# etiiiR/pixel-nerf

Measured on AMD Instinct MI355X. Metric: rays/sec (coarse+fine, 64+64 samples), higher is better.
Workload: dtype f32 (f16x3)

## Files before the change

### pixel-nerf_amd/csrc/mlp_dev.h

```cpp
#pragma once
#include "pnr_diag.h"
#include <cstddef>
#include <type_traits>

#include "mlp_layout.h"

namespace pnr {
namespace mlpk {

__device__ __forceinline__ f4 mfma(float a, float b, f4 c) {
    return __builtin_amdgcn_mfma_f32_16x16x4f32(a, b, c, 0, 0, 0);
}

typedef f4 Acc[RTW][CT];

__device__ __forceinline__ int opaque_lane(int lane) {
    asm volatile("" : "+v"(lane));
    return lane;
}

__device__ __forceinline__ void save_relu(const Acc &acc, float *slot, int64_t tile, int64_t n_points,
                                          int wave, int lane) {
    lane = opaque_lane(lane);
    const int g = lane >> 4, cl = lane & 15;
#pragma unroll
    for (int c = 0; c < CT; ++c) {
        const int64_t p = tile * COLS + 16 * c + cl;
        if (p >= n_points) continue;
#pragma unroll
        for (int r = 0; r < RTW; ++r) {
            const f4 v = acc[r][c];
            *reinterpret_cast<f4 *>(slot + p * H + 16 * (RTW * wave + r) + 4 * g) = relu4(v);
        }
    }
}

__device__ __forceinline__ void save_mask(const Acc &acc, uint32_t *mslot, int64_t tile, int64_t n_points,
                                          int wave, int lane) {
    static_assert(RTW == 4, "mask bytes assume 4 row tiles per wave");
    lane = opaque_lane(lane);
    const int g = lane >> 4, cl = lane & 15;
    auto nib = [](const f4 &v) {
        return (v.x > 0.f ? 1u : 0u) | (v.y > 0.f ? 2u : 0u) | (v.z > 0.f ? 4u : 0u) | (v.w > 0.f ? 8u : 0u);
    };
#pragma unroll
    for (int c = 0; c < CT; ++c) {
        const int64_t p = tile * COLS + 16 * c + cl;
        const uint32_t bits = nib(acc[0][c]) | (nib(acc[1][c]) << 4) | (nib(acc[2][c]) << 8) | (nib(acc[3][c]) << 12);
        if (p < n_points)
            *reinterpret_cast<uint16_t *>(reinterpret_cast<char *>(mslot) + p * 64 + 8 * wave + 2 * g) =
                (uint16_t)bits;
    }
}

template <int NK>
__device__ __forceinline__ void gemm(Acc &acc, const float *__restrict__ wp, const float *inb) {
    f4 A[RTW], B[CT];
#pragma unroll
    for (int r = 0; r < RTW; ++r) A[r] = *reinterpret_cast<const f4 *>(wp + r * 256);
#pragma unroll
    for (int c = 0; c < CT; ++c) B[c] = *reinterpret_cast<const f4 *>(inb + c * 16 * LDS_LD);
#pragma unroll 2
    for (int kb = 0; kb < NK; ++kb) {
        f4 An[RTW], Bn[CT];
        const int kn = kb + 1 < NK ? kb + 1 : kb;
#pragma unroll
        for (int r = 0; r < RTW; ++r)
            An[r] = *reinterpret_cast<const f4 *>(wp + (int64_t)kn * KB_FLOATS + r * 256);
#pragma unroll
        for (int c = 0; c < CT; ++c)
            Bn[c] = *reinterpret_cast<const f4 *>(inb + c * 16 * LDS_LD + kn * 16);
#pragma unroll
        for (int j = 0; j < 4; ++j)
#pragma unroll
            for (int c = 0; c < CT; ++c)
#pragma unroll
                for (int r = 0; r < RTW; ++r) acc[r][c] = mfma(A[r][j], B[c][j], acc[r][c]);
#pragma unroll
        for (int r = 0; r < RTW; ++r) A[r] = An[r];
#pragma unroll
        for (int c = 0; c < CT; ++c) B[c] = Bn[c];
    }
}

typedef float f8 __attribute__((ext_vector_type(8)));

__device__ __forceinline__ void split3(const f4 &lo, const f4 &hi, bf8 &x0, bf8 &x1, bf8 &x2) {
    const float x[8] = {lo.x, lo.y, lo.z, lo.w, hi.x, hi.y, hi.z, hi.w};
    u4 p0, p1, p2;
#pragma unroll
    for (int q = 0; q < 4; ++q) {
        unsigned a, b, c;
        split_pair(x[2 * q], x[2 * q + 1], a, b, c);
        p0[q] = a;
        p1[q] = b;
        p2[q] = c;
    }
    x0 = __builtin_bit_cast(bf8, p0);
    x1 = __builtin_bit_cast(bf8, p1);
    x2 = __builtin_bit_cast(bf8, p2);
}

__device__ __forceinline__ void lds_barrier() {
    asm volatile("s_waitcnt lgkmcnt(0)\n\ts_barrier" ::: "memory");
}

constexpr int A_DIST = 3;
constexpr int A_RING = A_DIST < 4 ? 4 : 8;

template <int NKS, int NTERM>
__device__ __forceinline__ void gemm_split(Acc &acc, const float *__restrict__ wp, const float *inbw,
                                           float *stg, int wave, int lane) {
    bf8 ra[A_RING][3];
    auto loadA = [&](bf8 (&dst)[3], int ks, int r) {
        const float *src = wp + (int64_t)ks * SKS_FLOATS + r * SRT_FLOATS;
#pragma unroll
        for (int q = 0; q < 3; ++q) dst[q] = *reinterpret_cast<const bf8 *>(src + q * 256);
    };
    auto split_own = [&](int ks, int buf) {
        const float *bp = inbw + 32 * ks;
        const f4 v = *reinterpret_cast<const f4 *>(bp);
        unsigned a0, a1, a2, b0, b1, b2;
        split_pair(v.x, v.y, a0, a1, a2);
        split_pair(v.z, v.w, b0, b1, b2);
        typedef unsigned u2 __attribute__((ext_vector_type(2)));
        float *d = stg + buf * STG_FLOATS + (wave % CT) * 768 + lane * 4 + 2 * (wave / CT);
        *reinterpret_cast<u2 *>(d) = u2{a0, b0};
        *reinterpret_cast<u2 *>(d + 256) = u2{a1, b1};
        *reinterpret_cast<u2 *>(d + 512) = u2{a2, b2};
    };
    split_own(0, 0);
#pragma unroll
    for (int r = 0; r < A_DIST; ++r) loadA(ra[r], 0, r);
    lds_barrier();
#pragma unroll 1
    for (int ks = 0; ks < NKS; ++ks) {
        const int kn = ks + 1 < NKS ? ks + 1 : ks;
        bf8 b0[CT], b1[CT], b2[CT];
        const float *sp = stg + (ks & 1) * STG_FLOATS + lane * 4;
#pragma unroll
        for (int c = 0; c < CT; ++c) {
            b0[c] = *reinterpret_cast<const bf8 *>(sp + c * 768);
            b1[c] = *reinterpret_cast<const bf8 *>(sp + c * 768 + 256);
            b2[c] = *reinterpret_cast<const bf8 *>(sp + c * 768 + 512);
        }
#pragma unroll
        for (int r = 0; r < RTW; ++r) {
            if (r == 1) split_own(kn, (ks + 1) & 1);
            const int rn = r + A_DIST;
            if (rn < RTW) loadA(ra[rn % A_RING], ks, rn);
            else loadA(ra[rn % A_RING], kn, rn - RTW);
            __builtin_amdgcn_sched_barrier(0);
            const bf8 *a = ra[r % A_RING];
#pragma unroll
            for (int c = 0; c < CT; ++c) {
                f4 v = acc[r][c];
                if (NTERM >= 9) {
                    v = mfma_bf(a[2], b2[c], v);
                    v = mfma_bf(a[1], b2[c], v);
                    v = mfma_bf(a[2], b1[c], v);
                }
                v = mfma_bf(a[2], b0[c], v);
                v = mfma_bf(a[1], b1[c], v);
                v = mfma_bf(a[0], b2[c], v);
                v = mfma_bf(a[1], b0[c], v);
                v = mfma_bf(a[0], b1[c], v);
                v = mfma_bf(a[0], b0[c], v);
                acc[r][c] = v;
            }
        }
        lds_barrier();
    }
}

typedef _Float16 h2 __attribute__((ext_vector_type(2)));
typedef float f2 __attribute__((ext_vector_type(2)));
typedef unsigned u2 __attribute__((ext_vector_type(2)));

__device__ __forceinline__ void split_f16x4(const f4 &v, float s, u2 &p0, u2 &p1) {
    const f2 a = {v.x * s, v.y * s}, b = {v.z * s, v.w * s};
    const unsigned a0 = __builtin_bit_cast(unsigned, __builtin_convertvector(a, h2));
    const unsigned b0 = __builtin_bit_cast(unsigned, __builtin_convertvector(b, h2));
    p0 = u2{a0, b0};
    p1 = u2{resid_pk(a0, a.x, a.y), resid_pk(b0, b.x, b.y)};
}

__device__ __forceinline__ int swz(int col, int k) {
    return 8 * ((k >> 3) ^ ((col >> 2) & 3)) + (k & 7);
}

template <int DIST, int NP = 2>
struct HRing {
    static constexpr int slots = DIST < RTW ? RTW : 2 * RTW;
    h8 ra[slots][NP];
};

template <int DIST, int NP>
__device__ __forceinline__ void hring_load(HRing<DIST, NP> &R, const float *__restrict__ wp, int slot, int ks, int r) {
    const float *src = wp + (int64_t)ks * sks_h_floats(NP) + r * srt_h_floats(NP);
    R.ra[slot][0] = *reinterpret_cast<const h8 *>(src);
    if constexpr (NP > 1) R.ra[slot][1] = *reinterpret_cast<const h8 *>(src + 256);
}

template <int DIST, int NKS = KS32, int NP = 2>
__device__ __forceinline__ void hring_prime(HRing<DIST, NP> &R, const float *__restrict__ wp) {
#pragma unroll
    for (int t = 0; t < DIST; ++t) hring_load(R, wp, t, (t / RTW) & (NKS - 1), t % RTW);
}

struct Fair {
    int *prog;
    int wave, it, mate;
};
template <int NKS, int DIST = H_DIST, int NP = 2>
__device__ __forceinline__ void gemm_f16_primed(Acc &acc, HRing<DIST, NP> &R, const float *__restrict__ wp,
                                                const _Float16 *pb0, const _Float16 *pb1, Fair *F = nullptr) {
    constexpr int H_RING = HRing<DIST, NP>::slots;
    static_assert(DIST < H_RING && H_RING % RTW == 0, "ring");
    constexpr int U = H_RING / RTW;
    static_assert(NKS % U == 0, "k-steps");
    static_assert((NKS & (NKS - 1)) == 0, "rotation mask");
    auto kstep = [&](int ks, auto ph_tag, auto tail_tag) {
        constexpr int ph = decltype(ph_tag)::value;
        constexpr bool tail = decltype(tail_tag)::value;
        h8 b0[CT], b1[CT];
        const int kr = ks & (NKS - 1);
#pragma unroll
        for (int c = 0; c < CT; ++c) {
            b0[c] = *reinterpret_cast<const h8 *>(pb0 + c * 16 * ROWH + 32 * kr);
            if constexpr (NP > 1) b1[c] = *reinterpret_cast<const h8 *>(pb1 + c * 16 * ROWH + 32 * kr);
        }
#pragma unroll
        for (int r = 0; r < RTW; ++r) {
            const int tn = ph * RTW + r + DIST;
            if (!tail || tn < U * RTW)
                hring_load(R, wp, tn % H_RING, (ks - ph + tn / RTW) & (NKS - 1), tn % RTW);
            __builtin_amdgcn_sched_barrier(0);
            const h8 *a = R.ra[(ph * RTW + r) % H_RING];
#pragma unroll
            for (int c = 0; c < CT; ++c) {
                f4 v = acc[r][c];
                if constexpr (NP > 1) {
                    v = mfma_h(a[1], b0[c], v);
                    v = mfma_h(a[0], b1[c], v);
                }
                v = mfma_h(a[0], b0[c], v);
                acc[r][c] = v;
            }
        }
    };
    auto iter = [&](int ks0, auto tail_tag) {
        if (F) {
            const int it = ++F->it;
            if (it > __builtin_amdgcn_readfirstlane(F->mate)) __builtin_amdgcn_s_setprio(0);
            else __builtin_amdgcn_s_setprio(1);
            F->prog[F->wave] = it;
            F->mate = F->prog[F->wave ^ 4];
        }
        kstep(ks0, std::integral_constant<int, 0>{}, tail_tag);
        if constexpr (U > 1) kstep(ks0 + 1, std::integral_constant<int, 1>{}, tail_tag);
    };
#pragma unroll 1
    for (int ks = 0; ks + U < NKS; ks += U) iter(ks, std::false_type{});
    iter(NKS - U, std::true_type{});
    if (F) __builtin_amdgcn_s_setprio(0);
}

template <int NKS, int DIST = H_DIST, int NP = 2>
__device__ __forceinline__ void gemm_f16(Acc &acc, const float *__restrict__ wp, const _Float16 *pb0,
                                         const _Float16 *pb1, Fair *F = nullptr) {
    HRing<DIST, NP> R;
    hring_prime<DIST, NKS, NP>(R, wp);
    gemm_f16_primed<NKS, DIST, NP>(acc, R, wp, pb0, pb1, F);
}

__device__ __forceinline__ void put_split4(_Float16 *P0, _Float16 *P1, int off, const f4 &v, float s) {
    u2 p0, p1;
    split_f16x4(v, s, p0, p1);
    *reinterpret_cast<u2 *>(P0 + off) = p0;
    *reinterpret_cast<u2 *>(P1 + off) = p1;
}

template <bool RELU = true>
__device__ __forceinline__ void relu_colmax(const Acc &acc, float *cmax, int wave, int lane) {
    lane = opaque_lane(lane);
    const int g = lane >> 4, cl = lane & 15;
#pragma unroll
    for (int c = 0; c < CT; ++c) {
        float m = 0.f;
#pragma unroll
        for (int r = 0; r < RTW; ++r) {
            f4 v = acc[r][c];
            if constexpr (!RELU) v = f4{fabsf(v.x), fabsf(v.y), fabsf(v.z), fabsf(v.w)};
            m = max3_nc(max3_nc(m, v.x, v.y), v.z, v.w);
        }
        m = rows_max(m);
        if (g == 0) cmax[(16 * c + cl) * 8 + wave] = m;
    }
}

__device__ __forceinline__ void put_split4_pair(_Float16 *Pl, int off, const f4 &v, float s) {
    u2 p0, p1;
    split_f16x4(v, s, p0, p1);
    const auto w0 = __builtin_amdgcn_permlane16_swap(p0.x, p1.x, false, false);
    const auto w1 = __builtin_amdgcn_permlane16_swap(p0.y, p1.y, false, false);
    typedef unsigned u4 __attribute__((ext_vector_type(4)));
    *reinterpret_cast<u4 *>(Pl + off) = u4{w0[0], w1[0], w0[1], w1[1]};
}
__device__ __forceinline__ void put_f16x4_pair(_Float16 *q, int off, const f4 &va, const f4 &vb, float s) {
    const f2 a0 = {va.x * s, va.y * s}, a1 = {va.z * s, va.w * s};
    const f2 b0 = {vb.x * s, vb.y * s}, b1 = {vb.z * s, vb.w * s};
    const u2 pa = {__builtin_bit_cast(unsigned, __builtin_convertvector(a0, h2)),
                   __builtin_bit_cast(unsigned, __builtin_convertvector(a1, h2))};
    const u2 pb = {__builtin_bit_cast(unsigned, __builtin_convertvector(b0, h2)),
                   __builtin_bit_cast(unsigned, __builtin_convertvector(b1, h2))};
    const auto w0 = __builtin_amdgcn_permlane16_swap(pa.x, pb.x, false, false);
    const auto w1 = __builtin_amdgcn_permlane16_swap(pa.y, pb.y, false, false);
    typedef unsigned u4 __attribute__((ext_vector_type(4)));
    *reinterpret_cast<u4 *>(q + off) = u4{w0[0], w1[0], w0[1], w1[1]};
}
template <bool RELU = true, int NP = 2>
__device__ __forceinline__ void relu_store_split(const Acc &acc, _Float16 *P0, _Float16 *P1,
                                                 const float *cmax, int *ecol, int wave, int lane,
                                                 int (&e_col)[CT]) {
    lane = opaque_lane(lane);
    const int g = lane >> 4, cl = lane & 15;
    _Float16 *Pl = (NP > 1 && (g & 1)) ? P1 : P0;
    const int kb = 16 * RTW * wave + 4 * (g & ~1);
    _Float16 *q0 = Pl + cl * ROWH + swz(cl, kb), *q1 = Pl + cl * ROWH + swz(cl, kb + 16);
#pragma unroll
    for (int c = 0; c < CT; ++c) {
        const int col = 16 * c + cl;
        const f4 m0 = *reinterpret_cast<const f4 *>(cmax + col * 8);
        const f4 m1 = *reinterpret_cast<const f4 *>(cmax + col * 8 + 4);
        e_col[c] = scale_exp(max3_nc(max3_nc(m0.x, m0.y, m0.z), max3_nc(m0.w, m1.x, m1.y), max_nc(m1.z, m1.w)));
    }
    if (wave == 0 && g == 0) {
#pragma unroll
        for (int c = 0; c < CT; ++c) ecol[16 * c + cl] = e_col[c];
    }
#pragma unroll
    for (int c = 0; c < CT; ++c) {
        const int col = 16 * c + cl;
        const float sc = __builtin_ldexpf(1.f, e_col[c]);
        if constexpr (NP == 1) {
            static_assert(RTW % 2 == 0, "row-tile pairs");
#pragma unroll
            for (int j = 0; j < RTW / 2; ++j) {
                const f4 va = RELU ? relu4(acc[2 * j][c]) : acc[2 * j][c];
                const f4 vb = RELU ? relu4(acc[2 * j + 1][c]) : acc[2 * j + 1][c];
                put_f16x4_pair((g & 1) ? q1 : q0, c * 16 * ROWH + j * 32, va, vb, sc);
            }
        } else {
#pragma unroll
        for (int r = 0; r < RTW; ++r) {
            const f4 v = acc[r][c];
            const f4 o = RELU ? relu4(v) : v;
            put_split4_pair((r & 1) ? q1 : q0, c * 16 * ROWH + (r >> 1) * 32, o, sc);
        }
        }
    }
}

__device__ __forceinline__ void load_bias(f4 (&b)[RTW], const float *__restrict__ bias, int wave, int lane) {
    const int g = opaque_lane(lane) >> 4;
#pragma unroll
    for (int r = 0; r < RTW; ++r) b[r] = *reinterpret_cast<const f4 *>(bias + 16 * (RTW * wave + r) + 4 * g);
}
__device__ __forceinline__ void set_bias(Acc &acc, const f4 (&b)[RTW], bool accumulate) {
#pragma unroll
    for (int r = 0; r < RTW; ++r)
#pragma unroll
        for (int c = 0; c < CT; ++c) acc[r][c] = accumulate ? acc[r][c] + b[r] : b[r];
}

__device__ __forceinline__ void add_bias(Acc &acc, const float *__restrict__ bias, int wave, int lane,
                                         bool accumulate) {
    const int g = opaque_lane(lane) >> 4;
#pragma unroll
    for (int r = 0; r < RTW; ++r) {
        const f4 b = *reinterpret_cast<const f4 *>(bias + 16 * (RTW * wave + r) + 4 * g);
#pragma unroll
        for (int c = 0; c < CT; ++c) acc[r][c] = accumulate ? acc[r][c] + b : b;
    }
}

__device__ __forceinline__ void store_relu(const Acc &acc, float *inbuf, int wave, int lane) {
    const int g = lane >> 4, cl = lane & 15;
#pragma unroll
    for (int r = 0; r < RTW; ++r)
#pragma unroll
        for (int c = 0; c < CT; ++c) {
            const f4 v = acc[r][c];
            const f4 o = relu4(v);
            *reinterpret_cast<f4 *>(inbuf + (16 * c + cl) * LDS_LD + 16 * (RTW * wave + r) + 4 * g) = o;
        }
}

#ifdef PNR_PHASE_TIMING
constexpr int PT_SLOTS = 20;
#endif

struct GemmCtx {
    int64_t wl_off, ws_off;
    const float *inb4;
    const float *inbw;
    float *stg;
    const float *hdr;
    const _Float16 *pb0, *pb1;
    const int *ecol;
    int ecl[CT];
    Fair fair;
    int wave, lane;
#ifdef PNR_PHASE_TIMING
    uint64_t pt[PT_SLOTS], pt_last;
#endif
};

struct CellRows {
    f4 c[2][4];
};
__device__ __forceinline__ void cell_load(CellRows &C, const float *__restrict__ pz, const float *gtab, int cj,
                                          int lane) {
    const f4 to = *reinterpret_cast<const f4 *>(gtab + cj * 8);
#pragma unroll
    for (int half = 0; half < 2; ++half) {
        const uint32_t ch = half * 256 + opaque_lane(lane) * 4;
        C.c[half][0] = *reinterpret_cast<const f4 *>(pz + __float_as_uint(to.x) + ch);
        C.c[half][1] = *reinterpret_cast<const f4 *>(pz + __float_as_uint(to.y) + ch);
        C.c[half][2] = *reinterpret_cast<const f4 *>(pz + __float_as_uint(to.z) + ch);
        C.c[half][3] = *reinterpret_cast<const f4 *>(pz + __float_as_uint(to.w) + ch);
    }
}
__device__ __forceinline__ void cell_blend_store(const CellRows &C, const float *gtab, float *stage, int cj,
                                                 int lane) {
    const f4 tw = *reinterpret_cast<const f4 *>(gtab + cj * 8 + 4);
#pragma unroll
    for (int half = 0; half < 2; ++half) {
        const uint32_t ch = half * 256 + opaque_lane(lane) * 4;
        const f4 *c = C.c[half];
        f4 zz;
#pragma unroll
        for (int q = 0; q < 4; ++q)
            zz[q] = add_rn(add_rn(add_rn(mul_rn(c[0][q], tw.x), mul_rn(c[1][q], tw.y)), mul_rn(c[2][q], tw.z)),
                           mul_rn(c[3][q], tw.w));
        *reinterpret_cast<f4 *>(stage + cj * LDS_LD + ch) = zz;
    }
}
__device__ __forceinline__ uint32_t cell_run_starts(const float *gtab, int c0) {
    uint32_t starts = 1u;
    uint32_t prev = __builtin_amdgcn_readfirstlane(__float_as_uint(gtab[c0 * 8]));
#pragma unroll
    for (int j = 1; j < COLS / WAVES; ++j) {
        const uint32_t k = __builtin_amdgcn_readfirstlane(__float_as_uint(gtab[(c0 + j) * 8]));
        if (k != prev) starts |= 1u << j;
        prev = k;
    }
    return starts;
}
__device__ __forceinline__ void stage_proj_runs(const float *__restrict__ pz, const float *gtab, float *stage,
                                                int wave, int lane) {
    constexpr int NC = COLS / WAVES;
    const int c0 = NC * wave;
    const uint32_t starts = cell_run_starts(gtab, c0);
    auto next = [&](int j) -> int {
        const uint32_t m = starts & ~((2u << j) - 1u);
        return m ? __builtin_ctz(m) : NC;
    };
    CellRows A, B, C;
    int a = 0, b = next(0), c = b < NC ? next(b) : NC;
    cell_load(A, pz, gtab, c0 + a, lane);
    if (b < NC) cell_load(B, pz, gtab, c0 + b, lane);
    if (c < NC) cell_load(C, pz, gtab, c0 + c, lane);
    lds_barrier();
    int j = 0;
    for (;;) {
        const int d = c < NC ? next(c) : NC;
        for (; j < b; ++j) cell_blend_store(A, gtab, stage, c0 + j, lane);
        if (j >= NC) break;
        if (d < NC) cell_load(A, pz, gtab, c0 + d, lane);
        const int e = d < NC ? next(d) : NC;
        for (; j < c; ++j) cell_blend_store(B, gtab, stage, c0 + j, lane);
        if (j >= NC) break;
        if (e < NC) cell_load(B, pz, gtab, c0 + e, lane);
        const int f = e < NC ? next(e) : NC;
        for (; j < d; ++j) cell_blend_store(C, gtab, stage, c0 + j, lane);
        if (j >= NC) break;
        if (f < NC) cell_load(C, pz, gtab, c0 + f, lane);
        a = d;
        b = e;
        c = f;
    }
}
template <bool HP>
__device__ __forceinline__ void stage_latent_gather(const float *__restrict__ latent, const float *gtab, float *image,
                                                    _Float16 *P0, _Float16 *P1, int *ecol, float *zsave,
                                                    int64_t n_valid, int wave, int lane) {
#pragma unroll 4
    for (int j = 0; j < COLS / WAVES; ++j) {
        const int cj = (COLS / WAVES) * wave + j;
        const f4 to = *reinterpret_cast<const f4 *>(gtab + cj * 8);
        const f4 tw = *reinterpret_cast<const f4 *>(gtab + cj * 8 + 4);
        f4 zh[2];
#pragma unroll
        for (int half = 0; half < 2; ++half) {
            const uint32_t ch = half * 256 + opaque_lane(lane) * 4;
            const f4 c0 = *reinterpret_cast<const f4 *>(latent + __float_as_uint(to.x) + ch);
            const f4 c1 = *reinterpret_cast<const f4 *>(latent + __float_as_uint(to.y) + ch);
            const f4 c2 = *reinterpret_cast<const f4 *>(latent + __float_as_uint(to.z) + ch);
            const f4 c3 = *reinterpret_cast<const f4 *>(latent + __float_as_uint(to.w) + ch);
            f4 zz;
#pragma unroll
            for (int q = 0; q < 4; ++q)
                zz[q] = add_rn(add_rn(add_rn(mul_rn(c0[q], tw.x), mul_rn(c1[q], tw.y)), mul_rn(c2[q], tw.z)),
                               mul_rn(c3[q], tw.w));
            if constexpr (HP) zh[half] = zz;
            else *reinterpret_cast<f4 *>(image + cj * LDS_LD + ch) = zz;
            if (zsave && cj < n_valid) *reinterpret_cast<f4 *>(zsave + (int64_t)cj * H + ch) = zz;
        }
        if constexpr (HP) {
            float m = 0.f;
#pragma unroll
            for (int hf = 0; hf < 2; ++hf)
                m = fmaxf(m, fmaxf(fmaxf(fabsf(zh[hf][0]), fabsf(zh[hf][1])), fmaxf(fabsf(zh[hf][2]), fabsf(zh[hf][3]))));
            m = wave_max(m);
            const int e = scale_exp(m);
            const float sc = __builtin_ldexpf(1.f, e);
            put_split4(P0, P1, cj * ROWH + swz(cj, lane * 4), zh[0], sc);
            put_split4(P0, P1, cj * ROWH + swz(cj, 256 + lane * 4), zh[1], sc);
            if (lane == 0) ecol[cj] = e;
        }
    }
}
__device__ __forceinline__ void add_stage(Acc &x, const float *stage, int wave, int lane) {
    lane = opaque_lane(lane);
    const int g = lane >> 4, cl = lane & 15;
#pragma unroll
    for (int r = 0; r < RTW; ++r)
#pragma unroll
        for (int c = 0; c < CT; ++c) {
            const f4 v = *reinterpret_cast<const f4 *>(stage + (16 * c + cl) * LDS_LD + 16 * (RTW * wave + r) + 4 * g);
            f4 o;
#pragma unroll
            for (int q = 0; q < 4; ++q) o[q] = add_rn(x[r][c][q], v[q]);
            x[r][c] = o;
        }
}

template <int PREC, int NK, int DIST = H_DIST, bool OWN = false, int NP = nparts(PREC)>
__device__ __forceinline__ void layer_gemm(Acc &acc, const float *layer_base, GemmCtx &g, int hidx,
                                           HRing<DIST, NP> *R = nullptr) {
    PT(g, 3);
    PT_COUNT(g, 5);
    if constexpr (PREC == 0) {
        gemm<NK>(acc, layer_base + g.wl_off, g.inb4);
    } else if constexpr (is_h(PREC)) {
        const int cl = opaque_lane(g.lane) & 15;
        const int ew = (int)g.hdr[HDR_ESCALE + hidx];
        float sa[CT], ia[CT];
#pragma unroll
        for (int c = 0; c < CT; ++c) {
            const int e = (OWN ? g.ecl[c] : g.ecol[16 * c + cl]) + ew;
            sa[c] = __builtin_ldexpf(1.f, e);
            ia[c] = __builtin_ldexpf(1.f, -e);
        }
#pragma unroll
        for (int r = 0; r < RTW; ++r)
#pragma unroll
            for (int c = 0; c < CT; ++c) {
                acc[r][c] *= sa[c];
            }
        Fair *F = g.fair.prog ? &g.fair : nullptr;
        const int wso = NP == nparts(PREC) ? (int)g.ws_off : RTW * g.wave * srt_h_floats(NP) + g.lane * 4;
        if (R) gemm_f16_primed<NK / 2, DIST, NP>(acc, *R, layer_base + opaque_lane(wso), g.pb0, g.pb1, F);
        else gemm_f16<NK / 2, DIST, NP>(acc, layer_base + opaque_lane(wso), g.pb0, g.pb1, F);
#pragma unroll
        for (int r = 0; r < RTW; ++r)
#pragma unroll
            for (int c = 0; c < CT; ++c) {
                acc[r][c] *= ia[c];
            }
    } else {
        gemm_split<NK / 2, PREC>(acc, layer_base + g.ws_off, g.inbw, g.stg, g.wave, g.lane);
    }
    PT(g, 2);
}

__device__ __forceinline__ int claim_one(int *p) {
    int old;
    unsigned long long saved;
    asm volatile(
        "s_mov_b64 %1, exec\n\t"
        "s_mov_b64 exec, 1\n\t"
        "s_nop 4\n\t"
        "global_atomic_add %0, %2, %3, off sc0\n\t"
        "s_mov_b64 exec, %1\n\t"
        "s_waitcnt vmcnt(0)\n\t"
        "s_nop 4"
        : "=&v"(old), "=&s"(saved)
        : "v"(p), "v"(1)
        : "memory");
    return __builtin_amdgcn_readfirstlane(old);
}

}
}
```

### pixel-nerf_amd/csrc/mlp_layout.h

```cpp
#pragma once
#include "pnr_common.h"

namespace pnr {
namespace mlpk {

constexpr int H = 512;
constexpr int NRT = H / 16;
constexpr int NKB = H / 16;
constexpr int NKB_IN = 4;
constexpr int WAVES = 8;
constexpr int NTHR = 64 * WAVES;
constexpr int RTW = NRT / WAVES;
constexpr int CT = 4;
constexpr int COLS = 16 * CT;
constexpr int LDS_LD = H + 4;
constexpr int KB_FLOATS = NRT * 256;
constexpr int LAYER_FLOATS = NKB * KB_FLOATS;
constexpr int HDR = 64;
constexpr int KS32 = H / 32;
constexpr int KS32_IN = 2;
constexpr int SRT_FLOATS = 768;
constexpr int SKS_FLOATS = NRT * SRT_FLOATS;
constexpr int SRT16_FLOATS = 512;
constexpr int SKS16_FLOATS = NRT * SRT16_FLOATS;
constexpr int HDR_ESCALE = 32;
__host__ __device__ constexpr bool is_h(int prec) { return prec == 3 || prec == 1; }
__host__ __device__ constexpr int nparts(int prec) { return prec == 1 ? 1 : 2; }
__host__ __device__ constexpr int srt_h_floats(int np) { return np * 256; }
__host__ __device__ constexpr int sks_h_floats(int np) { return NRT * srt_h_floats(np); }
static_assert(srt_h_floats(2) == SRT16_FLOATS && sks_h_floats(2) == SKS16_FLOATS, "two-part layout");
__host__ __device__ constexpr int sks_floats(int prec) {
    return prec == 3 ? SKS16_FLOATS : prec == 1 ? sks_h_floats(1) : SKS_FLOATS;
}
__host__ __device__ constexpr int sks_in_floats(int prec) { return is_h(prec) ? SKS16_FLOATS : SKS_FLOATS; }
constexpr int STG_FLOATS = CT * 3 * 256;
constexpr int ROWH = H + 16;
constexpr int PART_HALVES = COLS * ROWH;
constexpr int H_DIST = 4;

struct Layout {
    int prec;
    int n_linz, n_l512, n_blocks, ncomb, d_in, d_out, pe_n;
    int64_t layer_floats;
    int64_t off_lin_in, off_l512, off_lin_out, off_bias, nbias, off_out32, total;
};

inline Layout make_layout(const pnr_mlp_desc &d) {
    Layout L;
    L.n_blocks = d.n_blocks;
    L.n_linz = d.combine_layer < d.n_blocks ? d.combine_layer : d.n_blocks;
    L.ncomb = L.n_linz;
    L.n_l512 = L.n_linz + 2 * d.n_blocks;
    L.d_in = d.d_in;
    L.d_out = d.d_out;
    L.pe_n = d.pe_n;
    L.prec = d.precision;
    L.layer_floats = L.prec ? (int64_t)KS32 * sks_floats(L.prec) : (int64_t)LAYER_FLOATS;
    L.off_lin_in = HDR;
    L.off_l512 = L.off_lin_in + (L.prec ? (int64_t)KS32_IN * sks_in_floats(L.prec) : (int64_t)NKB_IN * KB_FLOATS);
    L.off_lin_out = L.off_l512 + (int64_t)L.n_l512 * L.layer_floats;
    L.off_bias = L.off_lin_out + (int64_t)NKB * 256;
    L.nbias = (int64_t)(1 + L.n_l512) * H + 16;
    L.off_out32 = ((L.off_bias + L.nbias + 63) / 64) * 64;
    L.total = L.off_out32 + (is_h(L.prec) ? 4 * H : 0);
    return L;
}

__host__ __device__ inline int layer_index(int blk, int kind, int n_linz) {
    return blk < n_linz ? 3 * blk + kind : 3 * n_linz + 2 * (blk - n_linz) + (kind - 1);
}

__host__ __device__ constexpr int64_t save_floats_per_point(int n_blocks) {
    return 64 + (int64_t)H * (2 + 2 * n_blocks) + 16 * (2 * n_blocks + 1);
}
__host__ __device__ constexpr int64_t save_mask_offset(int n_blocks, int64_t n_points) {
    return (64 + (int64_t)H * (2 + 2 * n_blocks)) * n_points;
}

__device__ __forceinline__ int scale_exp(float m) {
    if (!(m > 0.f) || !(m < 3.0e38f)) return 0;
    int e = 14 - __builtin_amdgcn_frexp_expf(m);
    return e < -64 ? -64 : (e > 40 ? 40 : e);
}

struct FwdLds {
    int stg, gtab, cmax, ecol, petab, s_next, prog, hpart, mreg, mscr, mnf, petab_f, end, ltab;
};
enum LeanTab { LT_END = 0, LT_LSTEP, LT_STEP, LT_PAD, LT_WLF, LT_HLF, LT_KX, LT_KY, LT_HX, LT_HY, LT_FLOATS = 16 };
constexpr int IMG_H_FLOATS = PART_HALVES;
constexpr int MARCH_BUF_FLOATS = 640;
constexpr FwdLds fwd_lds(bool hp) {
    FwdLds m = {};
    m.stg = COLS * LDS_LD;
    m.gtab = hp ? IMG_H_FLOATS : m.stg + 2 * STG_FLOATS;
    m.cmax = m.gtab + COLS * 8;
    m.ecol = m.cmax + COLS * 8;
    m.petab = hp ? m.ecol + COLS : m.gtab + COLS * 8;
    m.s_next = m.petab + 32;
    m.prog = m.petab + 40;
    m.hpart = m.petab + 64;
    m.mreg = hp ? m.hpart + WAVES * COLS * 4 : m.petab + 36;
    m.mscr = m.mreg + MARCH_BUF_FLOATS;
    m.mnf = m.mscr + 3 * 128;
    m.petab_f = m.mnf + 4;
    m.end = m.petab_f + 32;
    m.ltab = m.end;
    return m;
}
constexpr size_t lds_bytes(const FwdLds &m, bool march) { return sizeof(float) * (size_t)(march ? m.end : m.mreg); }
constexpr size_t lds_bytes_lean(const FwdLds &m) { return sizeof(float) * (size_t)(m.ltab + LT_FLOATS); }
constexpr int MARCH_LDS_FLOATS = fwd_lds(true).end - fwd_lds(true).mreg;

struct BwdLds {
    int cmax, ecol, prog, end;
};
constexpr BwdLds bwd_lds() {
    BwdLds m = {};
    m.cmax = IMG_H_FLOATS;
    m.ecol = m.cmax + COLS * 8;
    m.prog = m.ecol + COLS;
    m.end = m.prog + WAVES;
    return m;
}
constexpr size_t lds_bytes(const BwdLds &m) { return sizeof(float) * (size_t)m.end; }

static_assert(lds_bytes(fwd_lds(true), false) == 147968 && lds_bytes(fwd_lds(false), false) == 158864 &&
              lds_bytes(bwd_lds()) == 137504, "LDS totals");
static_assert(lds_bytes(fwd_lds(true), true) == 147968 + 4 * MARCH_LDS_FLOATS &&
              lds_bytes(fwd_lds(false), true) == 158864 + 4 * MARCH_LDS_FLOATS &&
              fwd_lds(false).end - fwd_lds(false).mreg == MARCH_LDS_FLOATS, "LDS totals with the march region");
static_assert(lds_bytes(fwd_lds(true), true) <= 160 * 1024 && lds_bytes(fwd_lds(false), true) <= 160 * 1024 &&
              lds_bytes(bwd_lds()) <= 160 * 1024, "one workgroup's LDS");
static_assert(lds_bytes_lean(fwd_lds(true)) == lds_bytes(fwd_lds(true), true) + 4 * LT_FLOATS &&
              lds_bytes_lean(fwd_lds(true)) <= 160 * 1024 && fwd_lds(true).ltab % 4 == 0,
              "the lean table fits beside the fp16 map and the march region, 16-byte aligned");
static_assert(sizeof(float) * COLS * LDS_LD <= 2 * sizeof(_Float16) * PART_HALVES,
              "the fp32 stage fits in the split image it aliases");

}
}
```

### pixel-nerf_amd/csrc/mlp_pack.hip

```cpp
#include "mlp_layout.h"
#include "pnr_launch.h"

namespace pnr {
namespace mlpk {

struct PackSrc {
    const float *lin_in_w, *lin_in_b, *lin_out_w, *lin_out_b, *pe_f, *pe_p;
    const float *w[24], *b[24];
};

__global__ void k_pack(PackSrc s, Layout L, float *__restrict__ out) {
    const int64_t i = (int64_t)blockIdx.x * blockDim.x + threadIdx.x;
    if (i >= L.total) return;
    float v = 0.0f;
    if (i < HDR) {
        if (i >= HDR_ESCALE && i < HDR_ESCALE + 1 + L.n_l512 && is_h(L.prec)) return;
        if (i < 16 && i < L.pe_n) v = s.pe_f[i];
        else if (i >= 16 && i < 32 && (i - 16) < L.pe_n) v = s.pe_p[i - 16];
    } else if (i < L.off_lin_out && L.prec) {
        return;
    } else if (i < L.off_l512) {
        const int e = (int)(i - L.off_lin_in);
        const int kb = e / KB_FLOATS, rt = (e / 256) % NRT, lane = (e >> 2) & 63, j = e & 3;
        const int row = 16 * rt + (lane & 15), col = 16 * kb + 4 * (lane >> 4) + j;
        if (col < L.d_in) v = s.lin_in_w[(int64_t)row * L.d_in + col];
    } else if (i < L.off_lin_out) {
        const int64_t r = i - L.off_l512;
        const int layer = (int)(r / LAYER_FLOATS);
        const int e = (int)(r % LAYER_FLOATS);
        const int kb = e / KB_FLOATS, rt = (e / 256) % NRT, lane = (e >> 2) & 63, j = e & 3;
        const int row = 16 * rt + (lane & 15), col = 16 * kb + 4 * (lane >> 4) + j;
        v = s.w[layer][(int64_t)row * H + col];
    } else if (i < L.off_bias) {
        const int e = (int)(i - L.off_lin_out);
        const int kb = e >> 8, lane = (e >> 2) & 63, j = e & 3;
        const int row = lane & 15, col = 16 * kb + 4 * (lane >> 4) + j;
        if (row < L.d_out) v = s.lin_out_w[(int64_t)row * H + col];
    } else if (i >= L.off_out32) {
        const int e = (int)(i - L.off_out32);
        const int ch = e >> 2, j = e & 3;
        if (j < L.d_out) v = s.lin_out_w[(int64_t)j * H + ch];
    } else {
        const int64_t r = i - L.off_bias;
        const int64_t nb = (int64_t)(1 + L.n_l512) * H;
        if (r < H) v = s.lin_in_b[r];
        else if (r < nb) v = s.b[r / H - 1][r % H];
        else if (r - nb < L.d_out) v = s.lin_out_b[r - nb];
    }
    out[i] = v;
}

__device__ __forceinline__ unsigned short bf16_rne(float x) {
    unsigned u = __float_as_uint(x);
    u += 0x7fffu + ((u >> 16) & 1u);
    return (unsigned short)(u >> 16);
}
__device__ __forceinline__ float bf16_to_f(unsigned short h) { return __uint_as_float((unsigned)h << 16); }

__global__ void k_pack_split(PackSrc s, Layout L, float *__restrict__ out) {
    const int64_t t = (int64_t)blockIdx.x * blockDim.x + threadIdx.x;
    const int64_t n_in = (int64_t)KS32_IN * NRT * 64;
    const int64_t n_l = (int64_t)KS32 * NRT * 64;
    if (t >= n_in + L.n_l512 * n_l) return;
    int layer, ks, rt, lane;
    float *dst;
    if (t < n_in) {
        layer = -1;
        ks = (int)(t / (NRT * 64)); rt = (int)((t / 64) % NRT); lane = (int)(t % 64);
        dst = out + L.off_lin_in + (int64_t)ks * SKS_FLOATS + rt * SRT_FLOATS + lane * 4;
    } else {
        const int64_t r = t - n_in;
        layer = (int)(r / n_l);
        const int64_t e = r % n_l;
        ks = (int)(e / (NRT * 64)); rt = (int)((e / 64) % NRT); lane = (int)(e % 64);
        dst = out + L.off_l512 + layer * L.layer_floats + (int64_t)ks * SKS_FLOATS + rt * SRT_FLOATS + lane * 4;
    }
    const int row = 16 * rt + (lane & 15);
    unsigned short p[3][8];
#pragma unroll
    for (int j = 0; j < 8; ++j) {
        const int col = 32 * ks + 8 * (lane >> 4) + j;
        float w = 0.f;
        if (layer < 0) { if (col < L.d_in) w = s.lin_in_w[(int64_t)row * L.d_in + col]; }
        else w = s.w[layer][(int64_t)row * H + col];
        const unsigned short h0 = bf16_rne(w);
        const float r1 = w - bf16_to_f(h0);
        const unsigned short h1 = bf16_rne(r1);
        const float r2 = r1 - bf16_to_f(h1);
        p[0][j] = h0; p[1][j] = h1; p[2][j] = bf16_rne(r2);
    }
#pragma unroll
    for (int q = 0; q < 3; ++q) {
        uint4 v;
        v.x = p[q][0] | ((unsigned)p[q][1] << 16); v.y = p[q][2] | ((unsigned)p[q][3] << 16);
        v.z = p[q][4] | ((unsigned)p[q][5] << 16); v.w = p[q][6] | ((unsigned)p[q][7] << 16);
        *reinterpret_cast<uint4 *>(dst + q * 256) = v;
    }
}

__global__ void k_layer_absmax(PackSrc s, Layout L, float *__restrict__ out) {
    const int layer = (int)blockIdx.y - 1;
    const float *w = layer < 0 ? s.lin_in_w : s.w[layer];
    const int64_t n = layer < 0 ? (int64_t)H * L.d_in : (int64_t)H * H;
    float m = 0.f;
    for (int64_t i = (int64_t)blockIdx.x * blockDim.x + threadIdx.x; i < n; i += (int64_t)gridDim.x * blockDim.x)
        m = fmaxf(m, fabsf(w[i]));
    m = wave_max(m);
    if ((threadIdx.x & 63) == 0)
        atomicMax(reinterpret_cast<unsigned *>(out + HDR_ESCALE + blockIdx.y), __float_as_uint(m));
}
__global__ void k_layer_escale(int n_slots, float *__restrict__ out) {
    const int i = threadIdx.x;
    if (i < n_slots) out[HDR_ESCALE + i] = (float)scale_exp(out[HDR_ESCALE + i]);
}

__global__ void k_pack_f16(PackSrc s, Layout L, float *__restrict__ out) {
    const int64_t t = (int64_t)blockIdx.x * blockDim.x + threadIdx.x;
    const int64_t n_in = (int64_t)KS32_IN * NRT * 64;
    const int64_t n_l = (int64_t)KS32 * NRT * 64;
    const int64_t n_all = n_in + L.n_l512 * n_l;
    if (t >= n_all) return;
    int layer, ks, rt, lane;
    float *dst;
    if (t < n_in) {
        layer = -1;
        ks = (int)(t / (NRT * 64)); rt = (int)((t / 64) % NRT); lane = (int)(t % 64);
        dst = out + L.off_lin_in + (int64_t)ks * SKS16_FLOATS + rt * SRT16_FLOATS + lane * 4;
    } else {
        const int64_t r = t - n_in;
        layer = (int)(r / n_l);
        const int64_t e = r % n_l;
        ks = (int)(e / (NRT * 64)); rt = (int)((e / 64) % NRT); lane = (int)(e % 64);
        dst = out + L.off_l512 + layer * L.layer_floats + (int64_t)ks * sks_floats(L.prec) +
              rt * srt_h_floats(nparts(L.prec)) + lane * 4;
    }
    const int np = layer < 0 ? 2 : nparts(L.prec);
    const int ew = (int)out[HDR_ESCALE + 1 + layer];
    const int row = 16 * rt + (lane & 15);
    _Float16 p[2][8];
#pragma unroll
    for (int j = 0; j < 8; ++j) {
        const int col = 32 * ks + 8 * (lane >> 4) + j;
        float w = 0.f;
        if (layer < 0) { if (col < L.d_in) w = s.lin_in_w[(int64_t)row * L.d_in + col]; }
        else w = s.w[layer][(int64_t)row * H + col];
        const float ws = __builtin_ldexpf(w, ew);
        const _Float16 h0 = (_Float16)ws;
        p[0][j] = h0;
        p[1][j] = (_Float16)(ws - (float)h0);
    }
#pragma unroll
    for (int q = 0; q < 2; ++q) {
        if (q >= np) break;
        typedef _Float16 h8t __attribute__((ext_vector_type(8)));
        h8t v = {p[q][0], p[q][1], p[q][2], p[q][3], p[q][4], p[q][5], p[q][6], p[q][7]};
        *reinterpret_cast<h8t *>(dst + q * 256) = v;
    }
}

__global__ void k_pack_f16_t(PackSrc s, Layout L, const float *__restrict__ hdr, float *__restrict__ out) {
    const int64_t t = (int64_t)blockIdx.x * blockDim.x + threadIdx.x;
    const int64_t n_l = (int64_t)KS32 * NRT * 64;
    if (t >= L.n_l512 * n_l) return;
    const int layer = (int)(t / n_l);
    const int64_t e = t % n_l;
    const int ks = (int)(e / (NRT * 64)), rt = (int)((e / 64) % NRT), lane = (int)(e % 64);
    float *dst = out + layer * L.layer_floats + (int64_t)ks * SKS16_FLOATS + rt * SRT16_FLOATS + lane * 4;
    const int ew = (int)hdr[HDR_ESCALE + 1 + layer];
    const int col = 16 * rt + (lane & 15);
    typedef _Float16 h8t __attribute__((ext_vector_type(8)));
    h8t p0, p1;
#pragma unroll
    for (int j = 0; j < 8; ++j) {
        const int row = 32 * ks + 8 * (lane >> 4) + j;
        const float ws = __builtin_ldexpf(s.w[layer][(int64_t)row * H + col], ew);
        const _Float16 h0 = (_Float16)ws;
        p0[j] = h0;
        p1[j] = (_Float16)(ws - (float)h0);
    }
    *reinterpret_cast<h8t *>(dst) = p0;
    *reinterpret_cast<h8t *>(dst + 256) = p1;
}

}

size_t mlp_packed_bytes(const pnr_mlp_desc &d) {
    return sizeof(float) * (size_t)mlpk::make_layout(d).total;
}

int mlp_check_desc(const pnr_mlp_desc &d) {
    if (d.d_hidden != mlpk::H || d.d_latent != mlpk::H)
        return fail(PNR_ERR_UNSUPPORTED, "fused MLP implements d_hidden = d_latent = 512 (got %d, %d)",
                    d.d_hidden, d.d_latent);
    if (d.d_out != 4) return fail(PNR_ERR_UNSUPPORTED, "d_out must be 4 (got %d)", d.d_out);
    if (d.n_blocks < 1 || d.n_blocks > 8) return fail(PNR_ERR_UNSUPPORTED, "n_blocks in [1, 8] (got %d)", d.n_blocks);
    if (d.combine_layer < 0) return fail(PNR_ERR_INVALID, "combine_layer < 0");
    if (d.pe_n < 0 || d.pe_n > 16) return fail(PNR_ERR_UNSUPPORTED, "pe_n in [0, 16] (got %d)", d.pe_n);
    if (d.d_in != 3 + 3 * d.pe_n + 3)
        return fail(PNR_ERR_UNSUPPORTED, "d_in must be 3 + 3*pe_n + 3 (xyz PE + raw viewdirs); got %d", d.d_in);
    if (d.d_in > 16 * mlpk::NKB_IN) return fail(PNR_ERR_UNSUPPORTED, "d_in <= 64");
    if (d.precision != PNR_PREC_F32 && d.precision != PNR_PREC_F16 && d.precision != PNR_PREC_F16X3 &&
        d.precision != PNR_PREC_BF16X6 && d.precision != PNR_PREC_BF16X9)
        return fail(PNR_ERR_UNSUPPORTED, "precision must be 0 (f32), 1 (f16, one product), 3 (f16x3) or 6 / 9 "
                    "(split bf16); got %d", d.precision);
    return PNR_OK;
}

static int pack_src(const pnr_mlp_weights &w, const mlpk::Layout &L, mlpk::PackSrc &s) {
    const pnr_mlp_desc &d = w.desc;
    s = {};
    s.lin_in_w = w.lin_in_w; s.lin_in_b = w.lin_in_b;
    s.lin_out_w = w.lin_out_w; s.lin_out_b = w.lin_out_b;
    s.pe_f = w.pe_freqs; s.pe_p = w.pe_phases;
    if (!s.lin_in_w || !s.lin_in_b || !s.lin_out_w || !s.lin_out_b || (d.pe_n && (!s.pe_f || !s.pe_p)))
        return fail(PNR_ERR_INVALID, "null weight pointer");
    for (int blk = 0; blk < d.n_blocks; ++blk) {
        for (int kind = 0; kind < 3; ++kind) {
            if (kind == 0 && blk >= L.n_linz) continue;
            const int li = mlpk::layer_index(blk, kind, L.n_linz);
            const float *wp = kind == 0 ? w.lin_z_w[blk] : kind == 1 ? w.fc0_w[blk] : w.fc1_w[blk];
            const float *bp = kind == 0 ? w.lin_z_b[blk] : kind == 1 ? w.fc0_b[blk] : w.fc1_b[blk];
            if (!wp || !bp) return fail(PNR_ERR_INVALID, "null weight pointer (block %d kind %d)", blk, kind);
            s.w[li] = wp;
            s.b[li] = bp;
        }
    }
    return PNR_OK;
}

int mlp_pack(const pnr_mlp_weights &w, void *packed, size_t bytes, hipStream_t st) {
    const pnr_mlp_desc &d = w.desc;
    int rc = mlp_check_desc(d);
    if (rc) return rc;
    mlpk::Layout L = mlpk::make_layout(d);
    if (bytes < sizeof(float) * (size_t)L.total) return fail(PNR_ERR_WORKSPACE, "packed buffer too small");
    mlpk::PackSrc s;
    if ((rc = pack_src(w, L, s))) return rc;
    const int64_t blocks = (L.total + 255) / 256;
    hipLaunchKernelGGL(mlpk::k_pack, dim3((unsigned)blocks), dim3(256), 0, st, s, L,
                       static_cast<float *>(packed));
    if (!launch_ok("mlp_pack")) return PNR_ERR_HIP;
    const int64_t n = (int64_t)(mlpk::KS32_IN + L.n_l512 * mlpk::KS32) * mlpk::NRT * 64;
    if (mlpk::is_h(L.prec)) {
        float *hdr = static_cast<float *>(packed);
        if (hipMemsetAsync(hdr + mlpk::HDR_ESCALE, 0, sizeof(float) * (1 + L.n_l512), st) != hipSuccess)
            return fail(PNR_ERR_HIP, "mlp_pack: hipMemsetAsync failed");
        hipLaunchKernelGGL(mlpk::k_layer_absmax, dim3(32, (unsigned)(1 + L.n_l512)), dim3(256), 0, st, s, L, hdr);
        if (!launch_ok("mlp_layer_absmax")) return PNR_ERR_HIP;
        hipLaunchKernelGGL(mlpk::k_layer_escale, dim3(1), dim3(64), 0, st, 1 + L.n_l512, hdr);
        if (!launch_ok("mlp_layer_escale")) return PNR_ERR_HIP;
        hipLaunchKernelGGL(mlpk::k_pack_f16, dim3((unsigned)((n + 255) / 256)), dim3(256), 0, st,
                           s, L, static_cast<float *>(packed));
        if (!launch_ok("mlp_pack_f16")) return PNR_ERR_HIP;
    } else if (L.prec) {
        hipLaunchKernelGGL(mlpk::k_pack_split, dim3((unsigned)((n + 255) / 256)), dim3(256), 0, st,
                           s, L, static_cast<float *>(packed));
        if (!launch_ok("mlp_pack_split")) return PNR_ERR_HIP;
    }
    return PNR_OK;
}

size_t mlp_packed_t_bytes(const pnr_mlp_desc &d) {
    if (mlp_check_desc(d) || d.precision != PNR_PREC_F16X3) return 0;
    const mlpk::Layout L = mlpk::make_layout(d);
    return sizeof(float) * (size_t)(L.n_l512 * L.layer_floats);
}

int mlp_pack_t(const pnr_mlp_weights &w, const void *packed, void *packed_t, size_t bytes, hipStream_t st) {
    const pnr_mlp_desc &d = w.desc;
    int rc = mlp_check_desc(d);
    if (rc) return rc;
    if (d.precision != PNR_PREC_F16X3)
        return fail(PNR_ERR_UNSUPPORTED, "the fused MLP backward implements precision 3 (f16x3); got %d", d.precision);
    const mlpk::Layout L = mlpk::make_layout(d);
    if (bytes < mlp_packed_t_bytes(d)) return fail(PNR_ERR_WORKSPACE, "transposed pack buffer too small");
    mlpk::PackSrc s;
    if ((rc = pack_src(w, L, s))) return rc;
    const int64_t n = (int64_t)L.n_l512 * mlpk::KS32 * mlpk::NRT * 64;
    hipLaunchKernelGGL(mlpk::k_pack_f16_t, dim3((unsigned)((n + 255) / 256)), dim3(256), 0, st, s, L,
                       static_cast<const float *>(packed), static_cast<float *>(packed_t));
    return launch_ok("mlp_pack_t") ? PNR_OK : PNR_ERR_HIP;
}

}
```

Baseline: 444,100.

## Permute hidden-dim k order so activation stores avoid permlane swaps

Introduces a k-slot permutation of the hidden dimension within each 32-row k-step and applies it both to packed weights (via kslot_inv at pack time) and to activation stores. Each lane group can then write its hi/lo f16 parts directly to P0/P1 as contiguous 16-byte chunks, with no permlane16_swap shuffles in relu_store_split. The latent input staging is remapped through kslot to match. This saves a few cross-lane ops per store but couples the weight packing layout to the activation layout, which must stay consistent.

```diff
diff --git a/pixel-nerf_amd/csrc/mlp_dev.h b/pixel-nerf_amd/csrc/mlp_dev.h
--- a/pixel-nerf_amd/csrc/mlp_dev.h
+++ b/pixel-nerf_amd/csrc/mlp_dev.h
@@ -299,35 +299,24 @@
     }
 }
 
-__device__ __forceinline__ void put_split4_pair(_Float16 *Pl, int off, const f4 &v, float s) {
-    u2 p0, p1;
-    split_f16x4(v, s, p0, p1);
-    const auto w0 = __builtin_amdgcn_permlane16_swap(p0.x, p1.x, false, false);
-    const auto w1 = __builtin_amdgcn_permlane16_swap(p0.y, p1.y, false, false);
+__device__ __forceinline__ void put_chunk(_Float16 *q, int off, const u2 &a, const u2 &b) {
     typedef unsigned u4 __attribute__((ext_vector_type(4)));
-    *reinterpret_cast<u4 *>(Pl + off) = u4{w0[0], w1[0], w0[1], w1[1]};
-}
-__device__ __forceinline__ void put_f16x4_pair(_Float16 *q, int off, const f4 &va, const f4 &vb, float s) {
-    const f2 a0 = {va.x * s, va.y * s}, a1 = {va.z * s, va.w * s};
-    const f2 b0 = {vb.x * s, vb.y * s}, b1 = {vb.z * s, vb.w * s};
-    const u2 pa = {__builtin_bit_cast(unsigned, __builtin_convertvector(a0, h2)),
-                   __builtin_bit_cast(unsigned, __builtin_convertvector(a1, h2))};
-    const u2 pb = {__builtin_bit_cast(unsigned, __builtin_convertvector(b0, h2)),
-                   __builtin_bit_cast(unsigned, __builtin_convertvector(b1, h2))};
-    const auto w0 = __builtin_amdgcn_permlane16_swap(pa.x, pb.x, false, false);
-    const auto w1 = __builtin_amdgcn_permlane16_swap(pa.y, pb.y, false, false);
-    typedef unsigned u4 __attribute__((ext_vector_type(4)));
-    *reinterpret_cast<u4 *>(q + off) = u4{w0[0], w1[0], w0[1], w1[1]};
+    *reinterpret_cast<u4 *>(q + off) = u4{a.x, a.y, b.x, b.y};
+}
+__device__ __forceinline__ u2 cvt_f16x4(const f4 &v, float s) {
+    const f2 a = {v.x * s, v.y * s}, b = {v.z * s, v.w * s};
+    return u2{__builtin_bit_cast(unsigned, __builtin_convertvector(a, h2)),
+              __builtin_bit_cast(unsigned, __builtin_convertvector(b, h2))};
 }
 template <bool RELU = true, int NP = 2>
 __device__ __forceinline__ void relu_store_split(const Acc &acc, _Float16 *P0, _Float16 *P1,
                                                  const float *cmax, int *ecol, int wave, int lane,
                                                  int (&e_col)[CT]) {
+    static_assert(RTW % 2 == 0, "row-tile pairs: a wave owns whole k-steps");
     lane = opaque_lane(lane);
     const int g = lane >> 4, cl = lane & 15;
-    _Float16 *Pl = (NP > 1 && (g & 1)) ? P1 : P0;
-    const int kb = 16 * RTW * wave + 4 * (g & ~1);
-    _Float16 *q0 = Pl + cl * ROWH + swz(cl, kb), *q1 = Pl + cl * ROWH + swz(cl, kb + 16);
+    const int kb = 16 * RTW * wave + 8 * g;
+    _Float16 *q0 = P0 + cl * ROWH + swz(cl, kb), *q1 = P1 + cl * ROWH + swz(cl, kb);
 #pragma unroll
     for (int c = 0; c < CT; ++c) {
         const int col = 16 * c + cl;
@@ -341,23 +330,21 @@
     }
 #pragma unroll
     for (int c = 0; c < CT; ++c) {
-        const int col = 16 * c + cl;
         const float sc = __builtin_ldexpf(1.f, e_col[c]);
-        if constexpr (NP == 1) {
-            static_assert(RTW % 2 == 0, "row-tile pairs");
-#pragma unroll
-            for (int j = 0; j < RTW / 2; ++j) {
-                const f4 va = RELU ? relu4(acc[2 * j][c]) : acc[2 * j][c];
-                const f4 vb = RELU ? relu4(acc[2 * j + 1][c]) : acc[2 * j + 1][c];
-                put_f16x4_pair((g & 1) ? q1 : q0, c * 16 * ROWH + j * 32, va, vb, sc);
+#pragma unroll
+        for (int j = 0; j < RTW / 2; ++j) {
+            const f4 va = RELU ? relu4(acc[2 * j][c]) : acc[2 * j][c];
+            const f4 vb = RELU ? relu4(acc[2 * j + 1][c]) : acc[2 * j + 1][c];
+            const int off = c * 16 * ROWH + j * 32;
+            if constexpr (NP == 1) {
+                put_chunk(q0, off, cvt_f16x4(va, sc), cvt_f16x4(vb, sc));
+            } else {
+                u2 a0, a1, b0, b1;
+                split_f16x4(va, sc, a0, a1);
+                split_f16x4(vb, sc, b0, b1);
+                put_chunk(q0, off, a0, b0);
+                put_chunk(q1, off, a1, b1);
             }
-        } else {
-#pragma unroll
-        for (int r = 0; r < RTW; ++r) {
-            const f4 v = acc[r][c];
-            const f4 o = RELU ? relu4(v) : v;
-            put_split4_pair((r & 1) ? q1 : q0, c * 16 * ROWH + (r >> 1) * 32, o, sc);
-        }
         }
     }
 }
@@ -526,8 +513,8 @@
             m = wave_max(m);
             const int e = scale_exp(m);
             const float sc = __builtin_ldexpf(1.f, e);
-            put_split4(P0, P1, cj * ROWH + swz(cj, lane * 4), zh[0], sc);
-            put_split4(P0, P1, cj * ROWH + swz(cj, 256 + lane * 4), zh[1], sc);
+            put_split4(P0, P1, cj * ROWH + swz(cj, kslot(lane * 4)), zh[0], sc);
+            put_split4(P0, P1, cj * ROWH + swz(cj, kslot(256 + lane * 4)), zh[1], sc);
             if (lane == 0) ecol[cj] = e;
         }
     }
diff --git a/pixel-nerf_amd/csrc/mlp_layout.h b/pixel-nerf_amd/csrc/mlp_layout.h
--- a/pixel-nerf_amd/csrc/mlp_layout.h
+++ b/pixel-nerf_amd/csrc/mlp_layout.h
@@ -36,6 +36,34 @@
 constexpr int STG_FLOATS = CT * 3 * 256;
 constexpr int ROWH = H + 16;
 constexpr int PART_HALVES = COLS * ROWH;
+__host__ __device__ constexpr int kslot(int rho) {
+    return (rho & ~31) | (((rho >> 2) & 3) << 3) | (((rho >> 4) & 1) << 2) | (rho & 3);
+}
+__host__ __device__ constexpr int kslot_inv(int p) {
+    return (p & ~31) | (((p >> 2) & 1) << 4) | (((p >> 3) & 3) << 2) | (p & 3);
+}
+namespace kslot_check {
+constexpr bool all(bool (*f)(int), int n) {
+    for (int i = 0; i < n; ++i)
+        if (!f(i)) return false;
+    return true;
+}
+constexpr bool inverse(int rho) { return kslot_inv(kslot(rho)) == rho && kslot(kslot_inv(rho)) == rho; }
+constexpr bool keeps_kstep(int rho) { return (kslot(rho) & ~31) == (rho & ~31); }
+constexpr bool keeps_quads(int rho) { return kslot(rho) == kslot(rho & ~3) + (rho & 3) && kslot(rho & ~3) % 4 == 0; }
+constexpr bool chunk_rows(int t) {
+    for (int i = 0; i < 4; ++i)
+        if (kslot_inv(8 * t + i) != 32 * (t >> 2) + 4 * (t & 3) + i ||
+            kslot_inv(8 * t + 4 + i) != 32 * (t >> 2) + 16 + 4 * (t & 3) + i)
+            return false;
+    return true;
+}
+static_assert(all(inverse, H), "kslot is a bijection with inverse kslot_inv");
+static_assert(all(keeps_kstep, H), "kslot permutes inside a k-step of 32 rows");
+static_assert(all(keeps_quads, H), "kslot keeps aligned groups of 4 rows consecutive");
+static_assert(all(chunk_rows, H / 8), "lane group G's chunk is rows 4G.. of both row tiles of the k-step");
+}
+
 constexpr int H_DIST = 4;
 
 struct Layout {
diff --git a/pixel-nerf_amd/csrc/mlp_pack.hip b/pixel-nerf_amd/csrc/mlp_pack.hip
--- a/pixel-nerf_amd/csrc/mlp_pack.hip
+++ b/pixel-nerf_amd/csrc/mlp_pack.hip
@@ -140,7 +140,8 @@
     _Float16 p[2][8];
 #pragma unroll
     for (int j = 0; j < 8; ++j) {
-        const int col = 32 * ks + 8 * (lane >> 4) + j;
+        const int pos = 32 * ks + 8 * (lane >> 4) + j;
+        const int col = layer < 0 ? pos : kslot_inv(pos);
         float w = 0.f;
         if (layer < 0) { if (col < L.d_in) w = s.lin_in_w[(int64_t)row * L.d_in + col]; }
         else w = s.w[layer][(int64_t)row * H + col];
@@ -172,7 +173,7 @@
     h8t p0, p1;
 #pragma unroll
     for (int j = 0; j < 8; ++j) {
-        const int row = 32 * ks + 8 * (lane >> 4) + j;
+        const int row = kslot_inv(32 * ks + 8 * (lane >> 4) + j);
         const float ws = __builtin_ldexpf(s.w[layer][(int64_t)row * H + col], ew);
         const _Float16 h0 = (_Float16)ws;
         p0[j] = h0;
```

After: 448,400 (median of 6 runs). Within noise of the previous version (+1.0%).
